# amirhajibabaei/AutoForce

Hardware: AMD Instinct MI355X
Metric: MD-step atoms*steps/sec (SGPR predict: NL + descriptors + K_nm + E/F/stress + covloss); `value`: a Langevin MD loop on the device, every step from the forces of the one before (sgpr_md_run; --steps dependent steps between two fences); `value_resident_frames`: steps over independent frames resident i (higher is better)
Workload: dtype f64

## Files before the change

autoforce_amd/csrc/api.hip:

```cpp
#include <math.h>
#include <stdarg.h>
#include <stdio.h>
#include <stdlib.h>
#include <string.h>

#include <algorithm>
#include <atomic>
#include <numeric>
#include <type_traits>

#include <dlfcn.h>
#include <unistd.h>
#include <rccl/rccl.h>

#include "../../include/sgpr_hip.h"
#include "sgpr_internal.h"
#include "nl_grid.inc"
#include <cmath>
#include <limits>

static thread_local char g_err[512] = "";
static int fail(int code, const char *fmt, ...)
{
    va_list ap;
// ... 140 lines not shown
    {
        if (p) (void)hipHostFree(p);
        p = dev = nullptr;
        n = 0;
    }
};

#define SGPR_PEER_MAX 16
struct PeerXchg {
    int world = 1, rank = 0;
    bool attached = false;
    size_t cap = 0;
    size_t bytes = 0, flag_off = 0;
    char *base = nullptr;
    char *peer_base[SGPR_PEER_MAX] = {};
    bool opened[SGPR_PEER_MAX] = {};
    unsigned epoch = 0;
    DevBuf<int> ctl;
    long long timeout_ticks = 3000000000LL;
    hipStream_t last_st = nullptr;
    bool any_st = false;
    hipEvent_t ev = nullptr;
    const double *slice(int parity, int r) const { return (const double *)base + ((size_t)parity * world + r) * cap; }
};

struct MdRun {
    int N = 0;
    std::vector<int32_t> numbers;
    std::vector<int> perm;
    int32_t pbc[3] = {1, 1, 1};
    int rank = 0, world = 1;
    long long t = 0;
    double hdt = 0.0, c1 = 1.0, dt = 0.0;
    int ring = 3;
    bool evaluated = false;
    bool started = false;
    std::vector<double> mass_sorted;
    struct Chain { bool ok = false; unsigned step = 0, bind = 0, opt = 0; long long t = 0; const double *pos = nullptr; } chain;
    struct Nh { bool on = false; double c1 = 0.0, c2 = 0.0, K0 = 0.0; } nh;
    struct Npt {
        bool on = false, started = false;
        NptParams par = {};
        double pfactor = 0.0;
        std::vector<double> cells;
        long long cells_first = 0;
    } npt;
    struct Relax { bool on = false, started = false; RelaxParams par = {}; } relax;
    struct Lbfgs { bool on = false; int mem = 0; double maxstep = 0.0, h0 = 0.0, damping = 0.0; long long base = 0; } lbfgs;
    struct Fix { int n = 0; std::vector<unsigned char> sorted; } fix;
    struct Filter {
        bool on = false;
        double shrink = 0.0;
        double s_host[6] = {0.0, 0.0, 0.0, 0.0, 0.0, 0.0};
    } filter;
    struct Meta {
        bool on = false, fresh = false;
        MetaPar par = {};
        int pace = 1;
        long long base = 0, pre = 0, cap = 0;
        int merge = 0;
        long long enq = 0;
        struct QlStage { bool set = false; double cut = 0.0; int nl = 0; int l[META_MAXD] = {0, 0, 0, 0, 0, 0}; } stage[META_MAXC];
        MetaQl ql = {};
        int nql = 0;
    } meta;
    struct Rec {
// ... 7 lines not shown
    struct VanHove {
        int every = 0, levels = 0, rbins = 0, tbins = 0, pbins = 0, dbins = 0, nch = 0, npairs = 0, split = 1, S = 0;
        bool images = false;
        RdfGeom g = {};
        double rmax = 0.0, dmax = 0.0, volume = 0.0;
        std::vector<int> nz;
    } vh;
    struct Adf { int every = 0, bins = 0, nch = 0, S = 0; bool lds = true; std::vector<int> nz; } adf;
    struct Sq { int every = 0, nq = 0, lags = 0, origin_every = 1, nch = 0, S = 0; bool narrow = false; std::vector<int> nz; } sq;
    struct Bcm {
        std::vector<struct sgpr_model *> members;
        std::vector<double> info;
        bool cell = false;
    } bcm;
    struct Rep {
        enum Kind { NONE, BAND, POLYMER } kind = NONE;
        int R = 0, width = 0;
        std::vector<double> info;
    } rep;
    struct Neb { bool on = false; NebCell cell = {}; } neb;
    struct Pimd { bool on = false; double kT = 0.0, wP2 = 0.0; } pimd;
    static long long meta_dep(long long n, long long pace) { return (n + pace - 1) / pace; }
    long long meta_slot(long long n) const { return meta.pre + meta_dep(n, meta.pace) - meta_dep(meta.base, meta.pace); }
    static long long rec_between(long long a, long long b, int every) { return (b + every - 1) / every - (a + every - 1) / every; }
};
static_assert(std::is_default_constructible<MdRun>::value && std::is_nothrow_move_assignable<MdRun>::value,
              "a run is plain values, replaced by assignment: no DevBuf or HostBuf in it (they live in MdState)");

struct MdState {
    bool active = false;
    unsigned long long seed = 0;
    MdRun run;
    DevBuf<double> X, V, P, KE, mass, sig, noise, noise_raw, cell;
    DevBuf<double> zeta;
    DevBuf<int> halt;
    HostBuf<int> halt_host;
    DevBuf<double> scal_d;
    HostBuf<double> scal_pin;
    HostBuf<int> mark;
    size_t scal_rows = 0;
    struct {
        DevBuf<char> ring;
        DevBuf<double> Q;
        DevBuf<double> cells_d;
    } npt;
    struct {
        DevBuf<double> state;
        DevBuf<double> ref;
        DevBuf<double> cells;
    } relax;
    struct LbfgsBufs {
        DevBuf<double> hist, work;
        bool held() const { return hist.p != nullptr; }
    } lbfgs;
    struct { DevBuf<unsigned char> mask; } fixed;
    struct {
        DevBuf<double> f, s, in;
        DevBuf<int> perm;
    } filter;
    struct MetaBufs {
        DevBuf<double> centre, rows;
        DevBuf<int> key;
        DevBuf<unsigned char> sel;
        DevBuf<double> tcentre, tcnt, tlast;
        DevBuf<int> tkey, tstamp, ctl;
        bool held() const { return rows.p != nullptr; }
// ... 54 lines not shown
        DevBuf<double> ends;
        DevBuf<double> sums;
        DevBuf<double> coef;
        DevBuf<char> par;
    } neb;
    struct {
        DevBuf<double> V;
        DevBuf<double> sums;
        DevBuf<double> tab;
        DevBuf<double> sq;
    } pimd;
    NptSlot *slot(long long n) const { return (NptSlot *)npt.ring.p + (n & 3); }
    const unsigned char *fix() const { return run.fix.n ? fixed.mask.p : nullptr; }
    MetaTab meta_tab(long long want) const
    {
        MetaTab tb;
        tb.centre = meta.tcentre.p; tb.key = meta.tkey.p; tb.cnt = meta.tcnt.p; tb.last = meta.tlast.p; tb.stamp = meta.tstamp.p;
        tb.ctl = meta.ctl.p; tb.ch = run.meta.merge; tb.want = (int)want;
        return tb;
    }
};

struct sgpr_model {
    int lmax, nmax, S, device;
    double eta, rc;
    std::vector<int> species;
    std::vector<double> radii;
    hipStream_t stream = nullptr, side = nullptr;
    ncclComm_t comm = nullptr;
    int comm_rank = 0, comm_world = 1;
    PeerXchg peer;
    DevBuf<double> d_xpacked;
    hipEvent_t ev_fork = nullptr, ev_join = nullptr;
    int D, Dc, Dpad, CS;
    std::vector<PackEntry> h_pack;
    DevBuf<PackEntry> d_pack;
    DevBuf<double> d_radii;
    int m = 0, m_pad = 0, m_rows = 0;
    std::vector<int32_t> env_zc, env_z;
    std::vector<int64_t> env_ptr;
    std::vector<double> env_r;
    std::vector<int> ind_perm;
    std::vector<int> ind_slot;
    std::vector<int> qoff;
    DevBuf<int> d_ind_slot, d_ind_nn, d_qoff;
    DevBuf<double> d_Pm, d_PmT, d_pm_norm, d_M, d_mu, d_choli;
    bool has_mu = false, has_choli = false, choli_lower = true;
    const double *rows_mu = nullptr;
    std::vector<double> mean_w, vscale;
    DevBuf<double> d_vs_sqrt;
    int N = 0, N_rows = 0, rank = 0, world = 1, cnt = 0, cnt_rows = 0;
    int pbc[3] = {1, 1, 1};
    std::vector<int> numbers, perm , slot_sorted, aoff ;
    double mean_energy = 0.0;
    DevBuf<int> d_perm, d_slot, d_aoff, d_lslot , d_lnn;
    DevBuf<double> d_pos_in, d_cell_in, d_pos;
    const double *last_cell = nullptr;
    int maxnn = 0, nn_max_seen = 0;
    bool warm = false;
    bool zero_copy_out = true;
    bool spin_wait = true;
    DevBuf<char> d_grid;
    DevBuf<int> d_bin_of, d_bin_count, d_nn, d_nbr_j, d_nbr_shift, d_stat;
    int bin_cap = 0;
    DevBuf<BinRec> d_b_rec;
    DevBuf<BinAux> d_b_aux;
// ... 574 lines not shown
    if (lane < 3 && *f.flag) f.pos0[3 * (size_t)i + lane] = f.pos[3 * (size_t)i + lane];
    if (lane == 3) {
        const double v = 1.0 - cs;
        packed[3 * (size_t)f.N + c] = f.has_beta ? sqrt(v > 0.0 ? v : 0.0) * vs : 0.0;
    }
}

__device__ __forceinline__ double md_deviate(unsigned long long seed, long long t, int atom, int comp)
{
    unsigned c0 = (unsigned)t, c1 = (unsigned)((unsigned long long)t >> 32), c2 = (unsigned)atom, c3 = (unsigned)comp;
    unsigned k0 = (unsigned)seed, k1 = (unsigned)(seed >> 32);
#pragma unroll
    for (int r = 0; r < 10; r++) {
        const unsigned long long p0 = (unsigned long long)0xD2511F53u * c0, p1 = (unsigned long long)0xCD9E8D57u * c2;
        const unsigned n0 = (unsigned)(p1 >> 32) ^ c1 ^ k0, n1 = (unsigned)p1, n2 = (unsigned)(p0 >> 32) ^ c3 ^ k1, n3 = (unsigned)p0;
        c0 = n0; c1 = n1; c2 = n2; c3 = n3;
        k0 += 0x9E3779B9u; k1 += 0xBB67AE85u;
    }
    const unsigned long long a = ((unsigned long long)c0 << 32) | c1, b = ((unsigned long long)c2 << 32) | c3;
    const double u1 = (double)((a >> 11) + 1ull) * (1.0 / 9007199254740992.0);
    const double u2 = (double)(b >> 11) * (1.0 / 9007199254740992.0);
    return sqrt(-2.0 * log(u1)) * cos(6.283185307179586 * u2);
}

__global__ void md_deviates_kernel(int N, int rows, unsigned long long seed, long long t0, double *out)
{
    const size_t n3 = (size_t)3 * N, tot = n3 * rows;
    for (size_t e = (size_t)blockIdx.x * blockDim.x + threadIdx.x; e < tot; e += (size_t)gridDim.x * blockDim.x) {
        const size_t r = e / n3, w = e - r * n3;
        out[e] = md_deviate(seed, t0 + (long long)r, (int)(w / 3), (int)(w % 3));
    }
}

__device__ __forceinline__ double md_nh_advance(const FinNext &x, bool held, double F, double ms, double xc, double v0, double xprev, double zeta,
                                                double &xn)
{
#pragma clang fp contract(off)
    const double dt = 2.0 * x.hdt;
    const double a = __ddiv_rn((dt * dt) * (held ? 0.0 : F), ms);
    double xp = xprev;
    if (x.nh_first) xp = (xc - dt * v0) + 0.5 * a;
    const double b = x.hdt * zeta;
    const double num = ((2.0 * xc) - xp * (1.0 - b)) + a;
    xn = __ddiv_rn(num, 1.0 + b);
    const double vnow = x.nh_first ? v0 : __ddiv_rn(xn - xp, 2.0 * dt);
    if (held) xn = xc;
    return held ? 0.0 : vnow;
}

__device__ __forceinline__ double md_row_mul(double v, const double (&c)[3])
{
#pragma clang fp contract(off)
    return (fin_quad_lane<0>(v) * c[0] + fin_quad_lane<1>(v) * c[1]) + fin_quad_lane<2>(v) * c[2];
}

__device__ __forceinline__ double md_npt_advance(const FinNext &x, double F, double ms, double qc, double qp, double v0, const double (&c_hinv)[3],
                                                 const double (&c_bm1)[3], const double (&c_bp1)[3], const double (&c_h)[3], const double (&c_hn)[3],
                                                 double &qn, double &xn)
{
#pragma clang fp contract(off)
    const double dt = 2.0 * x.hdt;
    const double a = __ddiv_rn((dt * dt) * F, ms);
    const double num = ((2.0 * qc) + md_row_mul(qp, c_bm1)) + md_row_mul(a, c_hinv);
    qn = md_row_mul(num, c_bp1);
    const double vcen = __ddiv_rn(md_row_mul(qn - qp, c_h), 2.0 * dt);
    const double vnow = x.nh_first ? v0 : vcen;
// ... 486 lines not shown
            long long t0 = 1LL << 62, t1 = 0;
            int cntw = 0;
            const int np = pass == 0 ? 6 : 3;
            for (int i = 0; i < h->cnt; i++) {
                const long long *w = st.data() + ((size_t)pass * N + i) * 8;
                if (w[0] <= 0 || w[np - 1] <= 0) continue;
                for (int k = 0; k + 1 < np; k++) d[k] += (double)(w[k + 1] - w[k]);
                t0 = std::min(t0, w[0]); t1 = std::max(t1, w[np - 1]);
                cntw++;
            }
            fprintf(stderr, "[sgpr stamps] %s: %d waves, cycles per phase:", pass == 0 ? "list+forward (sweep, sort, list out, tiles, c+spectrum)" : "reverse (dE/dc, pairs)", cntw);
            for (int k = 0; k + 1 < np; k++) fprintf(stderr, " %.0f", d[k] / std::max(cntw, 1));
            fprintf(stderr, "; first start -> last end %lld\n", t1 - t0);
            if (pass == 0) {
                double e[3] = {0, 0, 0};
                for (int i = 0; i < h->cnt; i++) {
                    const long long *w = st.data() + (size_t)i * 8;
                    if (w[0] <= 0 || w[5] <= 0) continue;
                    e[0] += (double)(w[3] - w[0]); e[1] += (double)(w[4] - w[3]); e[2] += (double)(w[5] - w[4]);
                }
                fprintf(stderr, "[sgpr stamps]    as a reuse step: list filter %.0f | c (radial, harmonics, MFMA) %.0f | spectrum + rows out %.0f\n",
                        e[0] / std::max(cntw, 1), e[1] / std::max(cntw, 1), e[2] / std::max(cntw, 1));
            }
        }
    }
    drop_graph(h);
    for (auto e : h->ev) (void)hipEventDestroy(e);
    if (h->comm) (void)g_rccl.CommDestroy(h->comm);
    (void)sgpr_peer_destroy(h);
    if (h->stream) (void)hipStreamDestroy(h->stream);
    if (h->side) (void)hipStreamDestroy(h->side);
    if (h->ev_fork) (void)hipEventDestroy(h->ev_fork);
    if (h->ev_join) (void)hipEventDestroy(h->ev_join);
    delete h;
}

static void balance_xcd_share(std::vector<int4> &b, int ncu, int slots, const std::vector<int4> *extra = nullptr, bool cov_first = false)
{
    auto len = [&](const int4 &t) {
        int l = t.w - t.z;
        const unsigned sidx = (unsigned)t.y >> 16;
        if (extra && sidx) l += (*extra)[sidx - 1].w - (*extra)[sidx - 1].z;
        return l;
    };
    auto cov = [&](const int4 &t) { return cov_first && ((t.x >> 16) & 1); };
    std::stable_sort(b.begin(), b.end(), [&](const int4 &p, const int4 &q) { return len(p) != len(q) ? len(p) > len(q) : cov(p) > cov(q); });
    if (ncu <= 1) return;
    std::vector<long long> load(ncu, 0);
    std::vector<int> order(ncu);
    for (int r = 0; r < slots && (size_t)(r + 1) * ncu <= b.size(); r++) {
        for (int c = 0; c < ncu; c++) order[c] = c;
        std::stable_sort(order.begin(), order.end(), [&](int p, int q) { return load[p] > load[q]; });
        std::vector<int4> round(b.begin() + (size_t)r * ncu, b.begin() + (size_t)(r + 1) * ncu);
        std::stable_sort(round.begin(), round.end(), [&](const int4 &p, const int4 &q) { return len(p) > len(q); });
        for (int k = 0; k < ncu; k++) {
            const int4 t = round[ncu - 1 - k];
            b[(size_t)r * ncu + order[k]] = t;
            load[order[k]] += len(t);
        }
    }
}

static size_t count_tiles(const sgpr_model *h, int kind, int bm)
{
    const int nrows = h->cnt, ncols = kind == 1 ? h->Dpad : h->m;
    const int nrt = (nrows + bm - 1) / bm, nct = (ncols + 63) / 64;
// ... 1335 lines not shown
        return fail(SGPR_E_OVERFLOW, "neighbour-list capacity exceeded (neighbours %d/%d, bin %d/%d, reverse index %d/%d); "
                    "results of the steps since the last check are invalid", stat[0], h->maxnn, stat[1], h->bin_cap,
                    stat[2], h->t_stride);
    }
    h->nn_max_seen = stat[0];
    return peer_check(h);
}

extern "C" int sgpr_set_option(sgpr_model *h, const char *name, int value)
{
    if (!h || !name) return fail(SGPR_E_INVALID, "sgpr_set_option: bad arguments");
    h->opt_gen++;
    if (!strcmp(name, "graph")) {
        h->use_graph = value != 0; drop_graph(h); h->lists_valid = false; return SGPR_OK;
    }
    if (!strcmp(name, "overlap")) { h->use_fork = value != 0; drop_graph(h); return SGPR_OK; }
    if (!strcmp(name, "cov_in_rev")) { h->cov_in_rev = value != 0; drop_graph(h); return SGPR_OK; }
    if (!strcmp(name, "spin_wait")) { h->spin_wait = value != 0; return SGPR_OK; }
    if (!strcmp(name, "gemm_fused")) { h->gemm_fused = value != 0; return SGPR_OK; }
    if (!strcmp(name, "fuse_next")) { h->fuse_next = value != 0; h->pre_valid = false; h->lists_valid = false; return SGPR_OK; }
    if (!strcmp(name, "zero_copy_out")) { h->zero_copy_out = value != 0; return SGPR_OK; }
    if (!strcmp(name, "reverse_scatter")) {
        h->force_scatter = value != 0; h->gather_ok = !h->force_scatter; h->warm = false; h->lists_valid = false; h->pre_valid = false;
        drop_graph(h);
        return SGPR_OK;
    }
    if (!strcmp(name, "ignore_unknown_species")) { h->ignore_unknown = value != 0; return SGPR_OK; }
    if (!strcmp(name, "md_committee_cell")) {
        if (!h->md.active) return fail(SGPR_E_INVALID, "sgpr_set_option: md_committee_cell belongs to a run: call sgpr_md_begin first");
        if (h->md.run.t != 0 || h->md.run.started) return fail(SGPR_E_INVALID, "sgpr_set_option: md_committee_cell: the run has started");
        h->md.run.bcm.cell = value != 0;
        return SGPR_OK;
    }
    if (!strcmp(name, "lone_atom_weight")) {
        if (value < 1) return fail(SGPR_E_INVALID, "sgpr_set_option: lone_atom_weight >= 1");
        if (h->m > 0 && (double)value != h->lone_w) return fail(SGPR_E_INVALID, "sgpr_set_option: lone_atom_weight is set before the inducing set");
        h->lone_w = (double)value;
        return SGPR_OK;
    }
    if (!strcmp(name, "qr_keep")) {
        if (value < 0 || value > 2) return fail(SGPR_E_INVALID, "sgpr_set_option: qr_keep is 0, 1 or 2");
        h->qr_keep_mode = value;
        for (auto &k : h->qr_keep) k.valid = false;
        return SGPR_OK;
    }
    if (!strcmp(name, "skin_milliangstrom")) {
        if (value < 0) return fail(SGPR_E_INVALID, "sgpr_set_option: negative skin");
        h->skin = 1e-3 * value;
        h->lists_valid = false;
        return SGPR_OK;
    }
    return fail(SGPR_E_INVALID, "sgpr_set_option: unknown option %s", name);
}

__global__ void local_extract_kernel(int g, int maxnn, const int *nn, const int *nbr_j, const int *nbr_shift,
                                     const double *pos, const double *cell, double *out_r, int *out_slot)
{
    const int t = blockIdx.x * blockDim.x + threadIdx.x;
    if (t >= nn[g]) return;
    const size_t e = (size_t)g * maxnn + t;
    const int j = nbr_j[e], code = nbr_shift[e];
    const double s0 = (double)(int)(int8_t)(code & 0xff), s1 = (double)(int)(int8_t)((code >> 8) & 0xff),
                 s2 = (double)(int)(int8_t)((code >> 16) & 0xff);
    for (int k = 0; k < 3; k++)
        out_r[3 * t + k] = pos[3 * (size_t)j + k] - pos[3 * (size_t)g + k] + (s0 * cell[k] + s1 * cell[3 + k] + s2 * cell[6 + k]);
    out_slot[t] = (code >> 24) & 0xff;
// ... 134 lines not shown
```

autoforce_amd/csrc/md_host.inc:

```
static int md_alloc(sgpr_model *h, int N)
{
    MdState &m = h->md;
    bool bad = false;
    bad |= m.X.alloc((size_t)12 * N); bad |= m.V.alloc((size_t)12 * N); bad |= m.P.alloc(4 * (size_t)sgpr_packed_len(N));
    bad |= m.KE.alloc((size_t)8 * N); bad |= m.mass.alloc(N); bad |= m.sig.alloc(N); bad |= m.cell.alloc(9);
    bad |= m.halt.alloc(4); bad |= m.zeta.alloc(8);
    if (bad) return fail(SGPR_E_NODEVICE, "sgpr_md_begin: device allocation failed");
    if (!m.halt_host.p && m.halt_host.alloc_mapped(16)) return fail(SGPR_E_NODEVICE, "sgpr_md_begin: no mapped host memory");
    return SGPR_OK;
}

static bool md_same_system(const sgpr_model *h, int N, const int32_t *numbers, const int32_t *pbc, int rank, int world)
{
    bool same = (N == h->N && h->rank == rank && h->world == world && (int)h->numbers.size() == N);
    for (int i = 0; i < N && same; i++) same = h->numbers[i] == numbers[i];
    for (int k = 0; k < 3 && same; k++) same = h->pbc[k] == (pbc ? (pbc[k] != 0) : 1);
    return same;
}

static int md_rebind(sgpr_model *h)
{
    const MdState &m = h->md;
    if (md_same_system(h, m.run.N, m.run.numbers.data(), m.run.pbc, m.run.rank, m.run.world)) return SGPR_OK;
    return sgpr_bind_system(h, m.run.N, m.run.numbers.data(), m.run.pbc, m.run.rank, m.run.world);
// ... 110 lines not shown
}

static unsigned md_due_levels(long long s, int levels, int *ndue)
{
    unsigned due = 0;
    int n = 0;
    for (int l = 0; l < levels && (s & ((1ll << l) - 1)) == 0; l++, n++) due |= 1u << l;
    if (ndue) *ndue = n;
    return due;
}

extern "C" int sgpr_md_begin(sgpr_model *h, int N, const int32_t *numbers, const double *positions, const double *cell,
                             const int32_t *pbc, const double *masses, const double *velocities, double dt,
                             double friction, double kT)
{
    if (!h) return fail(SGPR_E_INVALID, "sgpr_md_begin: bad arguments");
    MdState &m = h->md;
    m.active = false;
    if (N <= 0 || !numbers || !positions || !cell)
        return fail(SGPR_E_INVALID, "sgpr_md_begin: bad arguments");
    if (!(dt > 0.0) || friction < 0.0 || kT < 0.0) return fail(SGPR_E_INVALID, "sgpr_md_begin: dt > 0, friction >= 0, kT >= 0");
    HIPCHK(hipSetDevice(h->device));
    const int tr = peer_on(h) ? h->peer.rank : 0, tw = peer_on(h) ? h->peer.world : 1;
    int rc_ = md_same_system(h, N, numbers, pbc, tr, tw) ? SGPR_OK : sgpr_bind_system(h, N, numbers, pbc, tr, tw);
    if (rc_) return rc_;
    rc_ = md_alloc(h, N);
    if (rc_) return rc_;
    MdRun run;
    run.numbers.assign(numbers, numbers + N);
    run.perm = h->perm;
    for (int k = 0; k < 3; k++) run.pbc[k] = pbc ? (pbc[k] != 0) : 1;
    run.rank = tr; run.world = tw;
    run.N = N; run.dt = dt; run.hdt = 0.5 * dt; run.c1 = exp(-friction * dt);
    const double c2 = sqrt(1.0 - run.c1 * run.c1);
    std::vector<double> xs((size_t)3 * N), vs((size_t)3 * N, 0.0), ms(N), sg(N);
    for (int i = 0; i < N; i++) {
        const int c = h->perm[i];
        for (int k = 0; k < 3; k++) {
            xs[3 * (size_t)i + k] = positions[3 * (size_t)c + k];
            if (velocities) vs[3 * (size_t)i + k] = velocities[3 * (size_t)c + k];
        }
        ms[i] = masses ? masses[c] : 1.0;
        if (!(ms[i] > 0.0)) return fail(SGPR_E_INVALID, "sgpr_md_begin: mass of atom %d is not positive", c);
        sg[i] = friction > 0.0 ? c2 * sqrt(kT / ms[i]) : 0.0;
    }
    HIPCHK(hipMemcpy(m.X.p, xs.data(), sizeof(double) * 3 * N, hipMemcpyHostToDevice));
    HIPCHK(hipMemcpy(m.V.p, vs.data(), sizeof(double) * 3 * N, hipMemcpyHostToDevice));
    HIPCHK(hipMemcpy(m.mass.p, ms.data(), sizeof(double) * N, hipMemcpyHostToDevice));
    HIPCHK(hipMemcpy(m.sig.p, sg.data(), sizeof(double) * N, hipMemcpyHostToDevice));
    HIPCHK(hipMemcpy(m.cell.p, cell, sizeof(double) * 9, hipMemcpyHostToDevice));
    run.mass_sorted = std::move(ms);
    m.run = std::move(run);
    m.active = true;
    h->pre_valid = false;
    return SGPR_OK;
}

extern "C" int sgpr_md_fix(sgpr_model *h, const uint8_t *fixed3N)
{
    if (!h) return fail(SGPR_E_INVALID, "sgpr_md_fix: bad arguments");
    MdState &m = h->md;
    if (!m.active) return fail(SGPR_E_INVALID, "sgpr_md_fix: call sgpr_md_begin first");
    if (m.run.nh.on || m.run.npt.on || m.run.relax.on) return fail(SGPR_E_INVALID, "sgpr_md_fix: call it before sgpr_md_thermostat and sgpr_md_relax");
    if (m.run.neb.on) return fail(SGPR_E_INVALID, "sgpr_md_fix: call it before sgpr_md_neb");
    if (m.run.pimd.on) return fail(SGPR_E_UNSUPPORTED, "sgpr_md_fix: the run is a ring polymer (sgpr_md_pimd), which runs without a mask");
    if (m.run.t != 0 || m.run.started) return fail(SGPR_E_INVALID, "sgpr_md_fix: the run has started");
// ... 427 lines not shown
}

struct MdHalt { int k = -1, code = 0, done = 0; };
static int md_decode_halt(sgpr_model *h, unsigned step0, int enq, int final_eval, bool want_cells, MdHalt *out)
{
    MdState &m = h->md;
    const int hv = md_halt_step(m);
    MdHalt &r = *out;
    r.done = enq;
    if (hv != MD_HALT_NONE) {
        r.k = hv - (int)step0;
        if (r.k < 0 || r.k >= enq) return fail(SGPR_E_INVALID, "sgpr_md_run: inconsistent halt record (%d of %d)", r.k, enq);
        r.code = m.halt_host.p[1] == hv ? 2 : (m.halt_host.p[0] == hv ? 1 : 3);
        r.done = r.k + 1;
        m.run.t += r.k;
        if (r.code == 2) { h->warm = false; r.done -= 1; }
    } else
        m.run.t += final_eval ? enq - 1 : enq;
    if (want_cells) m.run.npt.cells.resize((size_t)SGPR_MD_CELL * (size_t)std::max(r.done, 0));
    return SGPR_OK;
}

static int md_upload_noise(sgpr_model *h, int nevals, const double *noise, hipStream_t st)
{
    MdState &m = h->md;
    if (!noise) return SGPR_OK;
    const size_t len = (size_t)nevals * 3 * m.run.N;
    if (m.noise.alloc(len) || m.noise_raw.alloc(len)) return fail(SGPR_E_NODEVICE, "sgpr_md_run: device allocation failed");
    HIPCHK(hipMemcpyAsync(m.noise_raw.p, noise, sizeof(double) * len, hipMemcpyHostToDevice, st));
    hipLaunchKernelGGL(md_sort_rows_kernel, dim3(1024), dim3(256), 0, st, m.run.N, nevals, h->d_perm.p, m.noise_raw.p, m.noise.p);
    return SGPR_OK;
}

static int md_reset_lists(sgpr_model *h, hipStream_t st)
{
    h->lists_valid = false;
    h->pre_valid = false;
    HIPCHK(hipMemsetAsync(h->d_bin_count.p, 0, 2 * SGPR_BIN_INTS * sizeof(int), st));
    return SGPR_OK;
}

static void md_fill_integrator(const MdState &m, int j, const double *noise_dev, bool pend0, FinNext &x)
{
    const int RG = m.run.ring, sl = (int)((m.run.t + j) % RG), sn = (sl + 1) % RG, sp = (sl + RG - 1) % RG;
    const size_t N3 = (size_t)3 * m.run.N;
    memset(&x, 0, sizeof(x));
    x.x_cur = m.X.p + N3 * sl; x.v_cur = m.V.p + N3 * sl;
    x.x_next = m.X.p + N3 * sn; x.v_next = m.V.p + N3 * sn;
    x.mass = m.mass.p; x.sig = m.sig.p; x.noise = noise_dev ? noise_dev + N3 * (size_t)j : nullptr;
    x.hdt = m.run.hdt; x.c1 = m.run.c1; x.pending = (j > 0 || pend0) ? 1 : 0;
    if (m.run.nh.on) {
        x.nh = 1; x.nh_first = (m.run.t + j) == 0 ? 1 : 0;
        x.x_prev = m.X.p + N3 * sp; x.v_now = m.V.p + N3 * sl;
        if (m.run.t + j > 0) x.v_cur = m.V.p + N3 * sp;
        x.nh_zeta = m.zeta.p + ((m.run.t + j) & 3);
    }
    x.seed = noise_dev ? 0ull : m.seed; x.t_index = m.run.t + j;
    x.ke_cur = m.KE.p + (size_t)2 * m.run.N * sl;
    x.halt = m.halt.p;
    if (m.run.filter.on) { x.filt_cur = m.filter.f.p + N3 * sl; x.filt_next = m.filter.f.p + N3 * sn; x.shrink = m.run.filter.shrink; }
}

static void md_fill_moving_cell(const MdState &m, int j, FinNext &x)
{
    const size_t N3 = (size_t)3 * m.run.N, RG = (size_t)m.run.ring, sl = (size_t)(m.run.t + j) % RG, sn = (sl + 1) % RG, sp = (sl + RG - 1) % RG;
    x.npt_cur = m.slot(m.run.t + j); x.npt_next = m.slot(m.run.t + j + 1);
    x.q_cur = m.npt.Q.p + N3 * sl; x.q_prev = m.npt.Q.p + N3 * sp; x.q_next = m.npt.Q.p + N3 * sn;
}

static void md_npt_cutoffs(sgpr_model *h) { NptParams &p = h->md.run.npt.par; p.rc_list = h->rc + (h->use_graph ? 0.0 : h->skin); p.rc_phys = h->rc; }

static void md_thermostat_launch(sgpr_model *h, int j, int step, const double *packed, hipStream_t st)
{
    const MdState &m = h->md;
    const int N = m.run.N, sl = (int)((m.run.t + j) % m.run.ring), n30 = (int)((m.run.t + j) & 0x3fffffff);
    double *ke = m.KE.p + (size_t)2 * N * sl, *row = m.scal_d.p + (size_t)SGPR_MD_SCAL * j;
    if (m.run.npt.on)
        hipLaunchKernelGGL(md_npt_kernel, dim3(1), dim3(256), 0, st, N, m.run.npt.par, (NptSlot *)m.npt.ring.p, m.zeta.p, ke, (const double *)(m.V.p + (size_t)3 * N * sl),
                           (const double *)m.mass.p, packed, (const double *)h->d_cell0.p, n30, (const int *)m.halt.p, step, row, m.npt.cells_d.p + (size_t)SGPR_MD_CELL * j,
                           m.run.filter.on ? (const double *)(m.filter.s.p + 6 * ((m.run.t + j) & 3)) : (const double *)nullptr,
                           m.run.filter.on ? m.filter.s.p + 6 * ((m.run.t + j + 1) & 3) : (double *)nullptr, m.run.filter.shrink);
    else if (m.run.nh.on)
        hipLaunchKernelGGL(md_nh_kernel, dim3(1), dim3(256), 0, st, N, ke, m.zeta.p, n30, m.run.dt, m.run.nh.c1, m.run.nh.c2, m.run.nh.K0, (const int *)m.halt.p, step, row);
}

static int md_warm(sgpr_model *h, const double *pos, const double *cell, double *packed, hipStream_t st)
{
    const int rc_ = h->warm ? SGPR_OK : run_checked(h, pos, cell, packed, st);
    if (!rc_) h->warm = true;
    return rc_;
// ... 401 lines not shown
    HIPCHK(hipMemcpyAsync(P.data(), m.bcm.P.p, sizeof(double) * K1 * plen, hipMemcpyDeviceToHost, st));
    HIPCHK(hipStreamSynchronize(st));
    HIPCHK(hipGetLastError());
    m.halt_host.p[0] = m.halt_host.p[1] = m.halt_host.p[2] = MD_HALT_NONE;
    HIPCHK(hipMemcpyAsync(m.halt.p, m.halt_host.p, 2 * sizeof(int), hipMemcpyHostToDevice, st));
    for (size_t e = 0; e < (size_t)3 * N; e++) {
        double acc = 0.0;
        for (int k = 0; k < K1; k++) acc = acc + w[k] * P[(size_t)k * plen + e];
        F[e] = acc;
    }
    return SGPR_OK;
}

static int md_committee_run(sgpr_model *h, int nevals, const double *noise, double ediff, int final_eval, double *scalars, int *evals_done,
                            int *halt_code)
{
    MdState &m = h->md;
    MdCall c;
    if (const int ro = md_call_open(h, ediff, evals_done, halt_code, c)) return ro;
    hipStream_t st = c.st;
    const int N = c.N, RG = m.run.ring, K = (int)m.run.bcm.members.size(), K1 = K + 1;
    const size_t plen = c.plen, N3 = (size_t)3 * N;
    for (int k = 0; k < K; k++) {
        const sgpr_model *mk = m.run.bcm.members[k];
        if (!(mk->m > 0 && mk->has_mu && mk->has_choli)) return fail(SGPR_E_NOMODEL, "sgpr_md_run: member %d of the committee has lost its weights", k);
        HIPCHK(hipStreamSynchronize(mk->stream));
    }
    m.run.started = true;
    MdBinIdentity guard(h);
    const bool cellrun = m.run.npt.on;
    if (const int rp = md_prepare_call(h, nevals, st, cellrun)) return rp;
    if (m.bcm.info_d.alloc((size_t)BCM_INFO * ((size_t)nevals + 1), false)) return fail(SGPR_E_NODEVICE, "sgpr_md_run: device allocation failed");
    if (const int ru = md_upload_noise(h, nevals, noise, st)) return ru;
    const int s0 = (int)(m.run.t % RG);
    const unsigned step_a = h->step_count;
    hipLaunchKernelGGL(md_record_kernel, dim3((3 * N + 255) / 256), dim3(256), 0, st, N, 0, (const int *)h->d_perm.p,
                       (const double *)(m.X.p + N3 * s0), (const double *)nullptr, (const double *)nullptr, m.bcm.x.p, (double *)nullptr,
                       (double *)nullptr, (const int *)m.halt.p, (int)step_a);
    if (cellrun) md_npt_cutoffs(h);
    const bool start = cellrun && !m.run.npt.started;
    auto cell_of = [&](long long n) -> const double * { return (cellrun && m.run.npt.started) ? m.slot(n)->h : m.cell.p; };
    if (const int rw = start ? SGPR_OK : md_warm(h, m.X.p + N3 * s0, cell_of(m.run.t), m.bcm.P.p + plen * K, st)) return rw;
    for (int k = 0; k < K; k++) {
        sgpr_model *mk = m.run.bcm.members[k];
        if (!md_same_system(mk, N, m.run.numbers.data(), m.run.pbc, 0, 1))
            if (const int rb = sgpr_bind_system(mk, N, m.run.numbers.data(), m.run.pbc, 0, 1)) return rb;
        if (const int rw = start ? SGPR_OK : md_warm(mk, m.bcm.x.p, cell_of(m.run.t), m.bcm.P.p + plen * k, st)) return rw;
    }
    if (start) {
        if (const int rs = md_npt_start(h, st, nevals)) return rs;
        for (int r = 2; r < 4; r++) HIPCHK(hipMemcpy(m.slot(r)->h, m.cell.p, 9 * sizeof(double), hipMemcpyDeviceToDevice));
    }
    for (int k = 0; k < K; k++)
        if (const int rl = md_reset_lists(m.run.bcm.members[k], st)) return rl;
    md_call_start(h, c);
    if (const int rl = md_reset_lists(h, st)) return rl;
    const unsigned step0 = c.step0; const double gate = c.gate;
    const bool pend0 = m.run.t > 0;
    const int rc_ = md_enqueue_ahead(h, nevals, st, &c.enq, [&](int j) -> int {
        const int sl = (int)((m.run.t + j) % RG);
        for (int k = 0; k < K; k++) {
            sgpr_model *mk = m.run.bcm.members[k];
            const int re = enqueue_step(mk, m.bcm.x.p, cell_of(m.run.t + j), m.bcm.P.p + plen * k, st, nullptr);
            if (re) return re;
            mk->lists_valid = true;
        }
        const int re = enqueue_step(h, m.X.p + N3 * sl, cell_of(m.run.t + j), m.bcm.P.p + plen * K, st, nullptr);
        if (re) return re;
        h->lists_valid = true;
        const int step = (int)(step0 + j);
        double *packed = m.P.p + plen * sl, *info = m.bcm.info_d.p + (size_t)BCM_INFO * j, *row = m.scal_d.p + (size_t)SGPR_MD_SCAL * j;
        hipLaunchKernelGGL(md_bcm_kernel, dim3(1), dim3(256), 0, st, N, K1, plen, (const double *)m.bcm.P.p, packed, info, gate, m.halt.p,
                           m.halt_host.dev, step, row, m.mark.dev + j);
        FinNext x;
        md_fill_integrator(m, j, noise ? m.noise.p : nullptr, pend0, x);
        x.step = step;
        const bool stay = final_eval && j == nevals - 1;
        if (cellrun) md_fill_moving_cell(m, j, x);
        hipLaunchKernelGGL(cellrun ? md_bcm_move_kernel<true> : md_bcm_move_kernel<false>, dim3((N + 63) / 64), dim3(256), 0, st, N, K1, plen,
                           (const double *)m.bcm.P.p, (const double *)info, packed, m.bcm.x.p, (const int *)h->d_perm.p, x, stay ? 1 : 0);
        hipLaunchKernelGGL(md_bcm_ke_kernel, dim3(1), dim3(256), 0, st, N, (const double *)(m.KE.p + (size_t)2 * N * sl), (const int *)m.halt.p,
                           step, row);
        md_thermostat_launch(h, j, step, packed, st);
        return SGPR_OK;
    });
    for (int k = 0; k < K; k++) m.run.bcm.members[k]->lists_valid = false;
    h->lists_valid = false;
    if (rc_) return rc_;
    MdHalt r;
    if (const int rc = md_call_close(h, c, final_eval, scalars, cellrun, &r)) return rc;
    if (r.code == 2)
        for (int k = 0; k < K; k++) m.run.bcm.members[k]->warm = false;
    if (r.done > 0) {
        m.run.bcm.info.assign(BCM_INFO, 0.0);
        HIPCHK(hipMemcpy(m.run.bcm.info.data(), m.bcm.info_d.p + (size_t)BCM_INFO * (r.done - 1), sizeof(double) * BCM_INFO, hipMemcpyDeviceToHost));
    }
    md_finish_call(h, r, scalars, m.run.nh.on, final_eval, evals_done, halt_code);
    return SGPR_OK;
}

typedef MdRun::Rep::Kind RepKind;
static const char *rep_attach_name(RepKind kind) { return kind == MdRun::Rep::BAND ? "sgpr_md_neb" : "sgpr_md_pimd"; }

static int md_replica_attach(sgpr_model *h, const char *who, RepKind kind, int R, int width, const double *x0)
{
    MdState &m = h->md;
    const size_t RN3 = (size_t)3 * m.run.N * (size_t)R;
    if (m.rep.X.alloc(RN3 * RLX_RING) || m.rep.P.alloc((size_t)sgpr_packed_len(m.run.N) * (size_t)R * RLX_RING))
// ... 323 lines not shown
    hipStream_t st = c.st;
    const int N = c.N;
    const size_t plen = c.plen;
    if (m.run.meta.on) {
        if (!md_gather_form(h))
            return fail(SGPR_E_UNSUPPORTED, "sgpr_md_run: the bias (sgpr_md_meta) runs in the gather form of the fused last kernel only (one rank, no graph "
                        "replay, no side-stream fork, a skin > 0): the host loop around calculate() serves this run");
        if (const int rq = md_meta_ql_fits(h, ": the host loop around calculate() serves this run")) return rq;
        const long long nd = (m.run.t + nevals - 1) / m.run.meta.pace * m.run.meta.pace;
        if (nd >= m.run.t && m.run.meta_slot(nd) >= m.run.meta.cap)
            return fail(SGPR_E_INVALID, "sgpr_md_run: %d evaluations from configuration %lld deposit hills up to row %lld; the bias holds %lld "
                        "(sgpr_md_meta again, with a larger capacity and the hills of sgpr_md_meta_hills)", nevals, m.run.t, m.run.meta_slot(nd), m.run.meta.cap);
        if (m.run.meta.merge) {
            int ctl[META_CTL_LEN];
            HIPCHK(hipMemcpyAsync(ctl, m.meta.ctl.p, sizeof(ctl), hipMemcpyDeviceToHost, st));
            HIPCHK(hipStreamSynchronize(st));
            m.run.meta.enq = ctl[META_CTL_DONE];
        }
        m.run.meta.fresh = false;
    }
    if (m.run.adf.every) {
        if (!md_gather_form(h))
            return fail(SGPR_E_UNSUPPORTED, "sgpr_md_run: the bond angles (sgpr_md_adf) read the step's neighbour list behind the gather form of the fused last "
                        "kernel only (one rank, no graph replay, no side-stream fork, a skin > 0): the frame record and workloads.AdfCounts serve this run");
        size_t bytes = 0;
        if (h->maxnn > 0 && !md_adf_waves(m.run.adf, h->maxnn, bytes))
            return fail(SGPR_E_UNSUPPORTED, "sgpr_md_run: the bond angles (sgpr_md_adf) keep a centre's neighbours in LDS; a list of up to %d entries per atom with "
                        "%d bins and %d species does not fit %d bytes", h->maxnn, m.run.adf.bins, m.run.adf.S, ADF_LDS_BYTES);
    }
    m.run.started = true;
    MdBinIdentity guard(h);
    if (const int rp = md_prepare_call(h, nevals, st, m.run.npt.on)) return rp;
    if (const int ru = md_upload_noise(h, nevals, noise, st)) return ru;
    const int RG = m.run.ring, s0 = (int)(m.run.t % RG);
    if (m.run.npt.on) md_npt_cutoffs(h);
    if (m.run.npt.on && !m.run.npt.started)
        if (const int rs = md_npt_start(h, st)) return rs;
    auto cell_of = [&](long long n) -> const double * { return m.run.npt.on ? m.slot(n)->h : m.cell.p; };
    if (const int rw = md_warm(h, m.X.p + (size_t)3 * N * s0, cell_of(m.run.t), m.P.p + plen * s0, st)) return rw;
    const bool chain = m.run.chain.ok && h->warm && h->step_count == m.run.chain.step && h->bind_gen == m.run.chain.bind && h->opt_gen == m.run.chain.opt &&
                       m.run.t == m.run.chain.t && m.run.chain.pos == m.X.p + (size_t)3 * N * s0;
    md_call_start(h, c);
    if (chain) {
        h->lists_valid = true;
        h->pre_valid = true; h->pre_pos = m.run.chain.pos; h->pre_cell = cell_of(m.run.t); h->pre_step = h->step_count;
    } else if (const int rl = md_reset_lists(h, st))
        return rl;
    const unsigned step0 = c.step0;
    const unsigned epoch0 = h->peer.epoch;
    const bool pend0 = m.run.t > 0;
    const int rc_ = md_enqueue_ahead(h, nevals, st, &c.enq, [&](int j) -> int {
        const int sl = (int)((m.run.t + j) % RG), sn = (sl + 1) % RG, sp = (sl + RG - 1) % RG;
        StepNext nx;
        nx.mode = 2;
        nx.pos_next = m.X.p + (size_t)3 * N * sn;
        FinNext &x = nx.md;
        md_fill_integrator(m, j, noise ? m.noise.p : nullptr, pend0, x);
        if (m.run.npt.on) {
            md_fill_moving_cell(m, j, x);
            nx.cell_next = x.npt_next->h;
            h->step_grid = &x.npt_cur->grid;
        }
        x.fixed = m.fix();
        x.ke_prev = j > 0 ? m.KE.p + (size_t)2 * N * sp : nullptr;
        x.packed_prev = j > 0 ? m.P.p + plen * sp : nullptr;
        x.ediff = c.gate;
        x.halt_host = m.halt_host.dev;
        x.scal_cur = m.scal_d.p + (size_t)SGPR_MD_SCAL * j; x.scal_prev = m.scal_d.p + (size_t)SGPR_MD_SCAL * (j > 0 ? j - 1 : 0);
        x.mark_cur = m.mark.dev + j;
        const int re = enqueue_step(h, x.x_cur, cell_of(m.run.t + j), m.P.p + plen * sl, st, &nx);
        if (re) return re;
        h->lists_valid = true;
        if (!h->pre_valid) return fail(SGPR_E_UNSUPPORTED, "sgpr_md_run: the fused last kernel is not available for this model / frame (sharded "
                                        "without the library's own exchange, graph capture or a zero skin)");
        md_thermostat_launch(h, j, (int)(step0 + j), m.P.p + plen * sl, st);
        if (m.run.rec.every && (m.run.t + j) % m.run.rec.every == 0) md_record_frame(h, j, (int)(step0 + j), st);
        return md_sample_due(h, j, (int)(step0 + j), st);
    });
    if (rc_) return rc_;
    const int enq = c.enq;
    if (enq > 0) {
        FinArgs f = {};
        f.N = N;
        const int sl = (int)((m.run.t + enq - 1) % RG);
        f.nx.mode = 3; f.nx.step = (int)(step0 + enq);
        f.nx.ke_prev = m.KE.p + (size_t)2 * N * sl; f.nx.packed_prev = m.P.p + plen * sl;
        f.nx.ediff = c.gate; f.nx.halt = m.halt.p; f.nx.halt_host = m.halt_host.dev;
        f.nx.scal_prev = m.scal_d.p + (size_t)SGPR_MD_SCAL * (enq - 1);
        hipLaunchKernelGGL(finalize_tail_kernel, dim3(2), dim3(256), 0, st, f);
    }
// ... 919 lines not shown
```

Before: 51.60 million.

## Pre-draw Langevin noise rows on a side stream, double-buffered

For Langevin runs seeded on the device, the Gaussian deviates for chunks of steps are now generated ahead of time by a kernel on the side stream into a two-chunk ring buffer. Each step then reads a precomputed noise row instead of computing the Box-Muller/Philox deviate inside the fused integrator kernel, and events order refills against reads. The aim is to take the RNG cost off the dependent step chain and overlap it with force evaluation. In exchange it adds extra memory (up to about 32 MB per chunk), extra event waits and launches, and the risk of contention on the side stream if that stream is also used for the fork path.

```diff
diff --git a/autoforce_amd/csrc/api.hip b/autoforce_amd/csrc/api.hip
--- a/autoforce_amd/csrc/api.hip
+++ b/autoforce_amd/csrc/api.hip
@@ -196,6 +196,7 @@
     int rank = 0, world = 1;
     long long t = 0;
     double hdt = 0.0, c1 = 1.0, dt = 0.0;
+    bool langevin = false;
     int ring = 3;
     bool evaluated = false;
     bool started = false;
@@ -269,6 +270,12 @@
     unsigned long long seed = 0;
     MdRun run;
     DevBuf<double> X, V, P, KE, mass, sig, noise, noise_raw, cell;
+    struct {
+        DevBuf<double> rows;
+        bool on = false;
+        int R = 0, nevals = 0;
+        long long t0 = 0;
+    } predraw;
     DevBuf<double> zeta;
     DevBuf<int> halt;
     HostBuf<int> halt_host;
@@ -389,6 +396,9 @@
     PeerXchg peer;
     DevBuf<double> d_xpacked;
     hipEvent_t ev_fork = nullptr, ev_join = nullptr;
+    hipEvent_t ev_drawn[2] = {nullptr, nullptr}, ev_read[2] = {nullptr, nullptr};
+    bool md_predraw = true;
+    int md_predraw_rows = 0;
     int D, Dc, Dpad, CS;
     std::vector<PackEntry> h_pack;
     DevBuf<PackEntry> d_pack;
@@ -1029,6 +1039,16 @@
     }
 }
 
+__global__ void md_deviates_sorted_kernel(int N, int rows, unsigned long long seed, long long t0, const int *perm, const double *sig, double *out)
+{
+    const size_t n3 = (size_t)3 * N, tot = n3 * rows;
+    for (size_t e = (size_t)blockIdx.x * blockDim.x + threadIdx.x; e < tot; e += (size_t)gridDim.x * blockDim.x) {
+        const size_t r = e / n3, w = e - r * n3;
+        const int i = (int)(w / 3), k = (int)(w - 3 * (size_t)i);
+        out[e] = sig[i] != 0.0 ? md_deviate(seed, t0 + (long long)r, perm[i], k) : 0.0;
+    }
+}
+
 __device__ __forceinline__ double md_nh_advance(const FinNext &x, bool held, double F, double ms, double xc, double v0, double xprev, double zeta,
                                                 double &xn)
 {
@@ -1581,6 +1601,10 @@
     if (h->side) (void)hipStreamDestroy(h->side);
     if (h->ev_fork) (void)hipEventDestroy(h->ev_fork);
     if (h->ev_join) (void)hipEventDestroy(h->ev_join);
+    for (int k = 0; k < 2; k++) {
+        if (h->ev_drawn[k]) (void)hipEventDestroy(h->ev_drawn[k]);
+        if (h->ev_read[k]) (void)hipEventDestroy(h->ev_read[k]);
+    }
     delete h;
 }
 
@@ -2982,6 +3006,12 @@
         h->md.run.bcm.cell = value != 0;
         return SGPR_OK;
     }
+    if (!strcmp(name, "md_predraw")) { h->md_predraw = value != 0; return SGPR_OK; }
+    if (!strcmp(name, "md_predraw_rows")) {
+        if (value < 0) return fail(SGPR_E_INVALID, "sgpr_set_option: md_predraw_rows >= 0");
+        h->md_predraw_rows = value;
+        return SGPR_OK;
+    }
     if (!strcmp(name, "lone_atom_weight")) {
         if (value < 1) return fail(SGPR_E_INVALID, "sgpr_set_option: lone_atom_weight >= 1");
         if (h->m > 0 && (double)value != h->lone_w) return fail(SGPR_E_INVALID, "sgpr_set_option: lone_atom_weight is set before the inducing set");
diff --git a/autoforce_amd/csrc/md_host.inc b/autoforce_amd/csrc/md_host.inc
--- a/autoforce_amd/csrc/md_host.inc
+++ b/autoforce_amd/csrc/md_host.inc
@@ -166,6 +166,7 @@
     for (int k = 0; k < 3; k++) run.pbc[k] = pbc ? (pbc[k] != 0) : 1;
     run.rank = tr; run.world = tw;
     run.N = N; run.dt = dt; run.hdt = 0.5 * dt; run.c1 = exp(-friction * dt);
+    run.langevin = friction > 0.0 && kT > 0.0;
     const double c2 = sqrt(1.0 - run.c1 * run.c1);
     std::vector<double> xs((size_t)3 * N), vs((size_t)3 * N, 0.0), ms(N), sg(N);
     for (int i = 0; i < N; i++) {
@@ -659,6 +660,77 @@
     return SGPR_OK;
 }
 
+
+static bool md_predraw_applies(const sgpr_model *h, const double *noise)
+{
+    const MdState &m = h->md;
+    return h->md_predraw && !noise && m.seed != 0ull && m.run.langevin && !m.run.nh.on && !m.run.npt.on;
+}
+
+static int md_predraw_fill(sgpr_model *h, int c)
+{
+    MdState &m = h->md;
+    const auto &p = m.predraw;
+    const size_t N3 = (size_t)3 * m.run.N;
+    const int rows = (int)std::min<long long>(p.R, (long long)p.nevals - (long long)c * p.R), half = c & 1;
+    const unsigned blocks = (unsigned)std::min<size_t>(1024, (N3 * (size_t)rows + 255) / 256);
+    hipLaunchKernelGGL(md_deviates_sorted_kernel, dim3(blocks), dim3(256), 0, h->side, m.run.N, rows, m.seed, p.t0 + (long long)c * p.R,
+                       (const int *)h->d_perm.p, (const double *)m.sig.p, m.predraw.rows.p + N3 * (size_t)p.R * half);
+    HIPCHK(hipEventRecord(h->ev_drawn[half], h->side));
+    return SGPR_OK;
+}
+
+static int md_predraw_open(sgpr_model *h, int nevals, const double *noise, hipStream_t st)
+{
+    MdState &m = h->md;
+    auto &p = m.predraw;
+    p.on = false;
+    if (!md_predraw_applies(h, noise)) return SGPR_OK;
+    if (!h->side) HIPCHK(hipStreamCreateWithFlags(&h->side, hipStreamNonBlocking));
+    for (int k = 0; k < 2; k++) {
+        if (!h->ev_drawn[k]) HIPCHK(hipEventCreateWithFlags(&h->ev_drawn[k], hipEventDisableTiming));
+        if (!h->ev_read[k]) HIPCHK(hipEventCreateWithFlags(&h->ev_read[k], hipEventDisableTiming));
+    }
+    const size_t N3 = (size_t)3 * m.run.N;
+    const long long fit = (long long)(((size_t)32 << 20) / (N3 * sizeof(double)));
+    p.R = h->md_predraw_rows > 0 ? h->md_predraw_rows : (int)std::max<long long>(8, std::min<long long>(nevals, fit));
+    p.nevals = nevals; p.t0 = m.run.t;
+    const int chunks = (nevals + p.R - 1) / p.R;
+    if (m.predraw.rows.alloc(N3 * (size_t)p.R * (size_t)std::min(chunks, 2), false)) return fail(SGPR_E_NODEVICE, "sgpr_md_run: device allocation failed");
+    HIPCHK(hipEventRecord(h->ev_read[0], st));
+    HIPCHK(hipStreamWaitEvent(h->side, h->ev_read[0], 0));
+    for (int c = 0; c < std::min(chunks, 2); c++)
+        if (const int rf = md_predraw_fill(h, c)) return rf;
+    p.on = true;
+    return SGPR_OK;
+}
+
+static int md_predraw_row(sgpr_model *h, int j, hipStream_t st, const double **row)
+{
+    const MdState &m = h->md;
+    const auto &p = m.predraw;
+    *row = nullptr;
+    if (!p.on) return SGPR_OK;
+    const int c = j / p.R, r = j - c * p.R;
+    if (r == 0) {
+        HIPCHK(hipStreamWaitEvent(st, h->ev_drawn[c & 1], 0));
+        if (c >= 1 && ((long long)c + 1) * p.R < p.nevals) {
+            HIPCHK(hipEventRecord(h->ev_read[(c - 1) & 1], st));
+            HIPCHK(hipStreamWaitEvent(h->side, h->ev_read[(c - 1) & 1], 0));
+            if (const int rf = md_predraw_fill(h, c + 1)) return rf;
+        }
+    }
+    *row = m.predraw.rows.p + (size_t)3 * m.run.N * ((size_t)p.R * (c & 1) + (size_t)r);
+    return SGPR_OK;
+}
+
+static int md_noise_row(sgpr_model *h, int j, const double *noise, hipStream_t st, const double **row)
+{
+    if (!noise) return md_predraw_row(h, j, st, row);
+    *row = h->md.noise.p + (size_t)3 * h->md.run.N * (size_t)j;
+    return SGPR_OK;
+}
+
 static int md_reset_lists(sgpr_model *h, hipStream_t st)
 {
     h->lists_valid = false;
@@ -667,14 +739,14 @@
     return SGPR_OK;
 }
 
-static void md_fill_integrator(const MdState &m, int j, const double *noise_dev, bool pend0, FinNext &x)
+static void md_fill_integrator(const MdState &m, int j, const double *noise_row, bool pend0, FinNext &x)
 {
     const int RG = m.run.ring, sl = (int)((m.run.t + j) % RG), sn = (sl + 1) % RG, sp = (sl + RG - 1) % RG;
     const size_t N3 = (size_t)3 * m.run.N;
     memset(&x, 0, sizeof(x));
     x.x_cur = m.X.p + N3 * sl; x.v_cur = m.V.p + N3 * sl;
     x.x_next = m.X.p + N3 * sn; x.v_next = m.V.p + N3 * sn;
-    x.mass = m.mass.p; x.sig = m.sig.p; x.noise = noise_dev ? noise_dev + N3 * (size_t)j : nullptr;
+    x.mass = m.mass.p; x.sig = m.sig.p; x.noise = noise_row;
     x.hdt = m.run.hdt; x.c1 = m.run.c1; x.pending = (j > 0 || pend0) ? 1 : 0;
     if (m.run.nh.on) {
         x.nh = 1; x.nh_first = (m.run.t + j) == 0 ? 1 : 0;
@@ -682,7 +754,7 @@
         if (m.run.t + j > 0) x.v_cur = m.V.p + N3 * sp;
         x.nh_zeta = m.zeta.p + ((m.run.t + j) & 3);
     }
-    x.seed = noise_dev ? 0ull : m.seed; x.t_index = m.run.t + j;
+    x.seed = noise_row ? 0ull : m.seed; x.t_index = m.run.t + j;
     x.ke_cur = m.KE.p + (size_t)2 * m.run.N * sl;
     x.halt = m.halt.p;
     if (m.run.filter.on) { x.filt_cur = m.filter.f.p + N3 * sl; x.filt_next = m.filter.f.p + N3 * sn; x.shrink = m.run.filter.shrink; }
@@ -1150,6 +1222,7 @@
     if (const int rp = md_prepare_call(h, nevals, st, cellrun)) return rp;
     if (m.bcm.info_d.alloc((size_t)BCM_INFO * ((size_t)nevals + 1), false)) return fail(SGPR_E_NODEVICE, "sgpr_md_run: device allocation failed");
     if (const int ru = md_upload_noise(h, nevals, noise, st)) return ru;
+    if (const int rd = md_predraw_open(h, nevals, noise, st)) return rd;
     const int s0 = (int)(m.run.t % RG);
     const unsigned step_a = h->step_count;
     hipLaunchKernelGGL(md_record_kernel, dim3((3 * N + 255) / 256), dim3(256), 0, st, N, 0, (const int *)h->d_perm.p,
@@ -1191,7 +1264,9 @@
         hipLaunchKernelGGL(md_bcm_kernel, dim3(1), dim3(256), 0, st, N, K1, plen, (const double *)m.bcm.P.p, packed, info, gate, m.halt.p,
                            m.halt_host.dev, step, row, m.mark.dev + j);
         FinNext x;
-        md_fill_integrator(m, j, noise ? m.noise.p : nullptr, pend0, x);
+        const double *nrow;
+        if (const int rn = md_noise_row(h, j, noise, st, &nrow)) return rn;
+        md_fill_integrator(m, j, nrow, pend0, x);
         x.step = step;
         const bool stay = final_eval && j == nevals - 1;
         if (cellrun) md_fill_moving_cell(m, j, x);
@@ -1581,6 +1656,7 @@
     MdBinIdentity guard(h);
     if (const int rp = md_prepare_call(h, nevals, st, m.run.npt.on)) return rp;
     if (const int ru = md_upload_noise(h, nevals, noise, st)) return ru;
+    if (const int rd = md_predraw_open(h, nevals, noise, st)) return rd;
     const int RG = m.run.ring, s0 = (int)(m.run.t % RG);
     if (m.run.npt.on) md_npt_cutoffs(h);
     if (m.run.npt.on && !m.run.npt.started)
@@ -1604,7 +1680,9 @@
         nx.mode = 2;
         nx.pos_next = m.X.p + (size_t)3 * N * sn;
         FinNext &x = nx.md;
-        md_fill_integrator(m, j, noise ? m.noise.p : nullptr, pend0, x);
+        const double *nrow;
+        if (const int rn = md_noise_row(h, j, noise, st, &nrow)) return rn;
+        md_fill_integrator(m, j, nrow, pend0, x);
         if (m.run.npt.on) {
             md_fill_moving_cell(m, j, x);
             nx.cell_next = x.npt_next->h;
```

Result: no change. 51.86 million (median of 4 runs) (+0.5%).
